# dcaustin33/intro_to_gaussian_splatting

Measured on AMD Instinct MI355X. Metric: Mpixels/sec forward raster (1M Gaussians, 1080p) + max |dpixel| vs CPU ref, higher is better.
Workload: dtype f32; 1 GPU; C3: synthetic 1M Gaussians, 1920x1080 (metric config); n_gaussians=1000000, width=1920, height=1080, tile=16, semantics=ref_cpu, layout=wh3, frames_in_flight=1, launch=one hipGraph replay per frame, frame_sync=speculative (GSX_FLAG_NO_SYNC), counts confirmed after the timed region, parallelism=1 GPU

## Files before the change

### intro_to_gaussian_splatting_amd/csrc/gsx_api.hip

```cpp
#include <float.h>
#include <math.h>
#include <stdarg.h>
#include <stdio.h>
#include <string.h>

#include "gsx_internal.h"
#ifdef GSX_TEST_HOOKS
#include "gsx_debug.h"
#endif

namespace {

thread_local char g_error[512] = "";

int fail(int code, const char *fmt, ...) {
    va_list ap;
    va_start(ap, fmt);
    vsnprintf(g_error, sizeof g_error, fmt, ap);
    va_end(ap);
    return code;
}

#define GSX_HIP(expr)                                                                               \
    do {                                                                                            \
// ... 85 lines not shown
                     bool &sampled) {
    uint32_t *k0 = (uint32_t *)(ws + c.keys0), *k1 = (uint32_t *)(ws + c.keys1);
    uint32_t *v0 = (uint32_t *)(ws + c.vals0), *v1 = (uint32_t *)(ws + c.vals1);
    uint32_t *counters = (uint32_t *)(ws + c.counters);
    const uint32_t *row_of = p.original_index ? (const uint32_t *)p.row_of_index : nullptr;
    const gsx::DepthRoute route = gsx::depth_sort_route(n, p.kept_hint);
    sampled = route != gsx::kDepthLsd;
    gsx::SortHints sh{nullptr, nullptr, nullptr, false};
    gsx::ScheduleHint sched_hint{nullptr, nullptr, nullptr, 0u};
    if (fh && p.hints && (route == gsx::kDepth256 || route == gsx::kDepthLsd) && n >= gsx::kSortSamples && p.grid.count() > 0 &&
        gsx::blend_splits_long_tiles(p.grid, p.semantics, p.generic)) {
        const gsx::HintsLayout hl = gsx::hints_layout(max_tiles_of(p.grid.width, p.grid.height, p.grid.tile),
                                                      max_axis_tiles_of(p.grid.width, p.grid.height, p.grid.tile));
        uint32_t *hdr = (uint32_t *)p.hints;
        sh = gsx::SortHints{hdr, (const uint32_t *)(p.hints + hl.splitters), (uint32_t *)(p.hints + hl.samples),
                            p.hints_valid && route == gsx::kDepth256};
        const bool exact = route == gsx::kDepth256 && gsx::knob("GSX_EXACT_SPLITTERS", 1) != 0;
        if (exact) sh.next_splitters = (uint32_t *)(p.hints + hl.splitters);
        fh->blend = gsx::BlendHints{hdr, exact ? nullptr : sh.samples, (uint32_t *)(p.hints + hl.splitters), (uint32_t *)(p.hints + hl.lens), 0u};
        fh->sched_region = (uint32_t *)(p.hints + hl.sched);
        if (p.hints_valid && p.schedule != 0 && p.grid.count() > 2048) {
            sched_hint = gsx::ScheduleHint{(const uint32_t *)(p.hints + hl.lens), (uint32_t *)(p.hints + hl.sched), hdr,
                                           (uint32_t)p.grid.count(), (uint32_t)p.grid.nwy()};
            fh->sched = sched_hint.sched;
        }
    }
    gsx::SampleHint presample;
    if (sampled && !sh.use && gsx::knob("GSX_PRESAMPLE", 1) != 0)
        presample = gsx::depth_presample(route, ws + c.temp, n, gsx::emit_chunk_sums(ws + c.temp, n, cap), row_of);
    GSX_HIP(gsx::launch_project_pack(camera, p.camera_device, in, n, p.grid, p.semantics, p.tight, p.small_batch, p.sh_degree, k0, (gsx::Record *)(ws + c.rec),
                                     (gsx::TileRect *)(ws + c.rect), counters,
                                     p.semantics != GSX_SEM_STD_3DGS ? (float4 *)(ws + c.bbox) : nullptr, sched_hint,
                                     c.temp_bytes >= (size_t)(n / GSX_BOUNDS_ROWS + 1) ? (uint8_t *)(ws + c.temp) : nullptr, s, presample));
    if (tm) tm->mark();
    if (sampled)
        GSX_HIP(gsx::sort_depth_sampled(route, ws + c.temp, k0, k1, v0, v1, n, p.kept_hint, counters + kCtrKept,
                                        counters + kCtrCulled, (const gsx::TileRect *)(ws + c.rect),
                                        (gsx::TileRect *)(ws + c.rrect), 0, gsx::emit_chunk_sums(ws + c.temp, n, cap), sh, s, row_of,
                                        presample.splitters != nullptr));
    else {
        const bool carry = p.grid.ntx <= 256 && p.grid.nty <= 256 && cap >= n && gsx::knob("GSX_LSD_CARRY", 1) != 0;
        GSX_HIP(gsx::sort_depth_compact(ws + c.temp, k0, k1, v0, v1, n, counters + kCtrKept, counters + kCtrCulled,
                                        (const gsx::TileRect *)(ws + c.rect), (gsx::TileRect *)(ws + c.rrect), s, sh.samples,
                                        carry ? (uint32_t *)(ws + c.tvals0) : nullptr,
                                        carry ? (uint32_t *)(ws + c.tvals1) : nullptr, row_of));
    }
    if (tm) tm->mark();
    order = v0;
    return GSX_OK;
}

int bin_pairs(const Plan &p, const Carve &c, char *ws, int64_t n, int64_t cap, const gsx::TileRect *rrect,
              const uint32_t *order, const uint32_t *m_dev, bool sums_ready, const gsx::BinCounts &bc,
              const gsx::LongTiles &lt, StageTimer *tm, hipStream_t s, const uint32_t *&sorted_vals) {
    uint2 *ranges = (uint2 *)(ws + c.ranges);
    GSX_HIP(gsx::emit_instances(ws + c.temp, rrect, order, m_dev, n, cap, p.grid, ws + c.tkeys0, (uint32_t *)(ws + c.tvals0),
                                ranges, bc, sums_ready, p.kept_hint, s));
    if (tm) tm->mark();
    if (p.grid.count() > 0)
        GSX_HIP(gsx::sort_instances(ws + c.temp, cap, p.grid, ws + c.tkeys0, ws + c.tkeys1, (uint32_t *)(ws + c.tvals0),
                                    (uint32_t *)(ws + c.tvals1), ranges, bc.d32, lt, &sorted_vals, s));
    return GSX_OK;
}

int read_counts(const Carve &c, char *ws, int64_t cap, bool on_device, uint32_t *redo, int64_t (&counts)[3], hipStream_t s) {
    counts[0] = counts[1] = counts[2] = 0;
    if (on_device) GSX_HIP(hipMemcpyAsync(counts, ws + c.counters + 16, 24, hipMemcpyDeviceToHost, s));
    if (redo) GSX_HIP(hipMemcpyAsync(redo, ws + c.redo, 4, hipMemcpyDeviceToHost, s));
    GSX_HIP(hipStreamSynchronize(s));
    if (counts[1] > cap)
        return fail(GSX_ERR_WORKSPACE_TOO_SMALL, "frame needs %lld tile instances, workspace holds %lld",
                    (long long)counts[1], (long long)cap);
    return GSX_OK;
}

int bin_and_blend(const Plan &p, const Carve &c, char *ws, int64_t n, int64_t cap, const gsx::TileRect *rrect,
                  const uint32_t *order, const uint32_t *m_dev, const uint32_t *culled_dev, bool sums_ready,
                  GsxFrameStats *stats, StageTimer &tm, hipStream_t s, const FrameHints &fh = FrameHints()) {
    uint32_t *counters = (uint32_t *)(ws + c.counters);
    int64_t *dev2 = (int64_t *)(counters + 4);
    uint2 *ranges = (uint2 *)(ws + c.ranges);
    bool counts_on_device = false, counts_in_host = false;
    bool redo_counted = false;
    const bool has_redo = p.stats_bytes >= offsetof(GsxFrameStats, n_redo) + sizeof(int64_t);
    if (p.plain && !stats) return fail(GSX_ERR_INVALID_ARGUMENT, "GSX_FLAG_PLAIN_FOOTPRINTS needs stats_host: n_redo must reach the caller");
    bool parts_marked = false;
    if (n == 0 && p.tile_counts && p.grid.count() > 0)
        GSX_HIP(gsx::launch_zero_words(p.tile_counts, (size_t)p.grid.count(), s));
    if (p.grid.count() > 0 && n == 0 && p.semantics == GSX_SEM_STD_3DGS) {
        tm.mark();
        GSX_HIP(gsx::launch_zero_words((uint32_t *)ranges, (size_t)p.grid.count() * 2, s));
        GSX_HIP(gsx::launch_blend((const gsx::Record *)(ws + c.rec), nullptr, (const uint32_t *)(ws + c.tvals0), ranges,
                                  p.grid, p.out, p.semantics, p.background, p.generic, make_clear_plan(p, false),
                                  gsx::LongTiles{nullptr, nullptr, 0u}, nullptr, gsx::BlendHints{nullptr, nullptr, nullptr, nullptr, 0u}, s));
    } else if (n == 0) {
        tm.mark();
        GSX_HIP(gsx::launch_clear(make_clear_plan(p, true), p.out.ptr, s));
    } else {
        gsx::BinCounts bc{dev2, nullptr, counters + kCtrPairs, counters + kCtrLong, (uint32_t *)(ws + c.redo), culled_dev, n};
        if (p.no_sync && stats) {
            void *alias = nullptr;
            if (hipHostGetDevicePointer(&alias, stats, 0) == hipSuccess && alias) {
                bc.stats2_host = (int64_t *)alias;
                counts_in_host = true;
            } else {
                (void)hipGetLastError();
            }
        }
        const bool split = p.split && cap > 0 && gsx::blend_splits_long_tiles(p.grid, p.semantics, p.generic);
        gsx::LongTiles lt{counters + kCtrLong, (uint32_t *)(ws + c.longs), split ? gsx::kMaxLongTiles : 0u};
        lt.redo = (uint32_t *)(ws + c.redo);
        if (fh.blend.lens) {
            lt.cost = fh.blend.lens;
            lt.header = fh.blend.header;
            lt.cost_pct = (uint32_t)gsx::knob("GSX_LONG_COST_PCT", 30);
            lt.stay_pct = (uint32_t)gsx::knob("GSX_LONG_STAY_PCT", 75);
            if (!fh.sched || lt.cost_pct == 0) lt.header = nullptr;
        }
        const uint32_t *sorted_vals = nullptr;
        const int rc = bin_pairs(p, c, ws, n, cap, rrect, order, m_dev, sums_ready, bc, lt, &tm, s, sorted_vals);
        if (rc != GSX_OK) return rc;
        counts_on_device = true;
        if (p.grid.count() == 0) {
            GSX_HIP(gsx::launch_clear(make_clear_plan(p, true), p.out.ptr, s));
        } else {
            if (p.tile_counts) GSX_HIP(gsx::launch_tile_counts(ranges, p.grid.count(), p.tile_counts, s));
            const uint32_t *sched = fh.sched;
            gsx::BlendHints bh = fh.blend;
            bh.xcd_sched = fh.sched ? 1u : 0u;
            if (!sched && cap > 0 && gsx::blend_uses_schedule(p.grid, p.semantics, p.generic, n, p.schedule)) {
                if (p.semantics == GSX_SEM_REF_CPU && gsx::knob("GSX_COLD_XCD_SCHED", 1) != 0) {
                    uint32_t *hdr = bh.header ? bh.header : (uint32_t *)(ws + c.sched_header);
                    uint32_t *region = (bh.header && fh.sched_region) ? fh.sched_region : (uint32_t *)(ws + c.sched);
                    if (!(bh.header && !fh.sched_region)) {
                        GSX_HIP(gsx::launch_tile_schedule_xcd(ranges, p.grid.count(), p.grid.nwy(), region, hdr, s));
                        sched = region;
                        bh.header = hdr;
                        bh.xcd_sched = 1u;
                    }
                }
                if (!sched) {
                    sched = (uint32_t *)(ws + c.sched);
                    GSX_HIP(gsx::launch_tile_schedule(ranges, p.grid.count(), (uint32_t *)(ws + c.sched), s));
                }
            }
            tm.mark();
            bh.plain = p.plain ? 1u : 0u;
            redo_counted = p.semantics == GSX_SEM_REF_CPU && p.grid.tile == 16 && !p.generic;
            const int64_t ntl = p.grid.count();
            bh.rank_last = (fh.sched && ntl > 7400 && ntl <= 8192 && (int64_t)cap >= 128 * ntl) ? 1u : 0u;
            if (gsx::knob("GSX_RANK_LAST", -1) >= 0) bh.rank_last = (uint32_t)gsx::knob("GSX_RANK_LAST", -1);
            if (p.n_parts > 1 && gsx::blend_in_parts(p.grid, p.semantics, p.generic)) {
                bool first = true;
                for (int k = 0; k < p.n_parts; ++k) {
                    const gsx::TileSpan span{p.part_axis, p.part_bounds[k], p.part_bounds[k + 1], first ? 1u : 0u, (uint32_t)k};
                    if (span.hi > span.lo || (first && k == p.n_parts - 1)) {
                        GSX_HIP(gsx::launch_blend((const gsx::Record *)(ws + c.rec), (const float4 *)(ws + c.bbox), sorted_vals,
                                                  ranges, p.grid, p.out, p.semantics, p.background, p.generic,
                                                  make_clear_plan(p, false), lt, sched, bh, s, &span));
                        first = false;
                    }
                    GSX_HIP(hipEventRecord((hipEvent_t)p.part_events[k], s));
                }
                parts_marked = true;
            } else {
                GSX_HIP(gsx::launch_blend((const gsx::Record *)(ws + c.rec), (const float4 *)(ws + c.bbox), sorted_vals,
                                          ranges, p.grid, p.out, p.semantics, p.background, p.generic,
                                          make_clear_plan(p, false), lt, sched, bh, s));
            }
            tm.mark();
        }
    }
    if (!parts_marked)
        for (int k = 0; k < p.n_parts; ++k) GSX_HIP(hipEventRecord((hipEvent_t)p.part_events[k], s));
    if (p.no_sync) {
        if (stats) {
            if (!counts_on_device) {
                stats->n_visible = 0;
                stats->n_instances = 0;
                stats->n_kept = 0;
            } else if (!counts_in_host) {
                GSX_HIP(hipMemcpyAsync(stats, dev2, 16, hipMemcpyDeviceToHost, s));
                GSX_HIP(hipMemcpyAsync(&stats->n_kept, dev2 + 2, 8, hipMemcpyDeviceToHost, s));
            }
            if (has_redo) {
                stats->n_redo = 0;
                if (redo_counted) GSX_HIP(hipMemcpyAsync(&stats->n_redo, ws + c.redo, 4, hipMemcpyDeviceToHost, s));
            }
            stats->n_tiles = p.grid.count();
            stats->reserved = cap;
        }
        return GSX_OK;
    }
    int64_t host2[3];
    uint32_t redo_host = 0;
    const int rc = read_counts(c, ws, cap, counts_on_device, redo_counted ? &redo_host : nullptr, host2, s);
    if (rc != GSX_OK && rc != GSX_ERR_WORKSPACE_TOO_SMALL) return rc;
    if (stats) {
        stats->n_visible = host2[0];
        stats->n_instances = host2[1];
        stats->n_kept = host2[2];
        if (has_redo) stats->n_redo = redo_host;
        stats->n_tiles = p.grid.count();
        stats->reserved = 0;
    }
    tm.finish(stats);
    return rc;
}

#ifdef GSX_TEST_HOOKS
thread_local float g_backward_ms[3] = {0.0f, 0.0f, 0.0f};
#endif

struct GeometryGrads {
    float *means3d, *scales, *quats;
};

int render_backward(const GsxCamera *camera, const float *means3d, const float *scales, const float *quats,
                    const float *opacity_logit, const float *colors, int64_t n, int32_t tile_size, const float *image,
                    const float *grad_image, float *grad_colors, float *grad_opacity_logit, const GeometryGrads *geo,
                    const GsxParams *params, void *workspace, size_t workspace_bytes, void *stream) {
    hipStream_t s = (hipStream_t)stream;
    if (!camera) return fail(GSX_ERR_INVALID_ARGUMENT, "camera is NULL");
    Plan p;
    int rc = make_plan_or_fail(camera->width, camera->height, tile_size, const_cast<float *>(image), params, p);
    if (rc != GSX_OK) return rc;
    if (p.semantics != GSX_SEM_REF_CPU) return fail(GSX_ERR_INVALID_ARGUMENT, "gsx_render_backward supports GSX_SEM_REF_CPU only");
    if (p.sh) return fail(GSX_ERR_INVALID_ARGUMENT, "gsx_render_backward takes RGB colours, not GsxParams.sh");
    if (p.grid.wx0 != 0 || p.grid.wy0 != 0 || p.grid.wx1 != p.grid.ntx || p.grid.wy1 != p.grid.nty)
        return fail(GSX_ERR_INVALID_ARGUMENT, "gsx_render_backward renders the whole frame: no tile window");
    if (p.out.x0 != 0 || p.out.y0 != 0 || p.out.w != camera->width || p.out.h != camera->height)
        return fail(GSX_ERR_INVALID_ARGUMENT, "gsx_render_backward takes the whole frame: no output window");
    if (p.n_parts > 0) return fail(GSX_ERR_INVALID_ARGUMENT, "gsx_render_backward does not take substrips");
    if (params && (params->flags & GSX_FLAG_NO_SYNC)) return fail(GSX_ERR_INVALID_ARGUMENT, "gsx_render_backward synchronises: no GSX_FLAG_NO_SYNC");
    if (p.camera_device) return fail(GSX_ERR_INVALID_ARGUMENT, "gsx_render_backward reads the camera argument: no camera_device");
    rc = check_inputs(p, n, means3d, scales, quats, opacity_logit, colors);
    if (rc != GSX_OK) return rc;
    if (!grad_image || !grad_colors || !grad_opacity_logit) return fail(GSX_ERR_INVALID_ARGUMENT, "grad_image / grad_colors / grad_opacity_logit is NULL");
    Carve c;
    int64_t cap;
    rc = check_workspace(workspace, workspace_bytes, n, max_tiles_of(camera->width, camera->height, tile_size), c, cap,
                         geo ? kCarveGeometry : kCarveBackward);
    if (rc != GSX_OK) return rc;
    char *ws = (char *)workspace;
    StageTimer tm;
    tm.begin(p.timing, s);
    GSX_HIP(gsx::launch_zero_words((uint32_t *)grad_colors, (size_t)n * 3, s));
    GSX_HIP(gsx::launch_zero_words((uint32_t *)grad_opacity_logit, (size_t)n, s));
    if (geo) {
        GSX_HIP(gsx::launch_zero_words((uint32_t *)geo->means3d, (size_t)n * 3, s));
        GSX_HIP(gsx::launch_zero_words((uint32_t *)geo->scales, (size_t)n * 3, s));
        GSX_HIP(gsx::launch_zero_words((uint32_t *)geo->quats, (size_t)n * 4, s));
    }
    if (n == 0 || p.grid.count() == 0) {
        GSX_HIP(hipStreamSynchronize(s));
        return GSX_OK;
    }
    const gsx::GaussiansIn in{means3d, scales, quats, opacity_logit, colors, p.original_index, nullptr};
    const uint32_t *order;
    bool sampled;
    rc = project_and_sort(p, c, ws, *camera, in, n, cap, nullptr, nullptr, s, order, sampled);
    if (rc != GSX_OK) return rc;
    uint32_t *counters = (uint32_t *)(ws + c.counters);
    const gsx::TileRect *rrect = (const gsx::TileRect *)(ws + c.rrect);
    const gsx::BinCounts bcnt{(int64_t *)(counters + 4), nullptr, counters + kCtrPairs, counters + kCtrLong,
                              (uint32_t *)(ws + c.redo), counters + kCtrCulled, n};
    const gsx::LongTiles lt{counters + kCtrLong, (uint32_t *)(ws + c.longs), 0u};
    const uint32_t *sorted_vals = nullptr;
    rc = bin_pairs(p, c, ws, n, cap, rrect, order, counters + kCtrKept, sampled, bcnt, lt, nullptr, s, sorted_vals);
    if (rc != GSX_OK) return rc;
// ... 447 lines not shown
```

### intro_to_gaussian_splatting_amd/csrc/gsx_binning.hip

```cpp

#include "gsx_internal.h"
#include "gsx_schedule_device.h"

namespace gsx {
namespace {

constexpr int kBlock = 256;
constexpr int kPerThread = 4;
constexpr int kChunk = kBlock * kPerThread;
static_assert(kChunk == kEmitChunk, "gsx_plan.h sizes the chunk sums with this");
constexpr int kSelfScanChunks = 2048;

__device__ __forceinline__ void load_rects(const TileRect *__restrict__ rrect, uint32_t first, uint32_t m,
                                           TileRect (&r)[kPerThread]) {
    if (first + kPerThread <= m) {
        const uint4 *src = reinterpret_cast<const uint4 *>(rrect + first);
        const uint4 a = src[0], b = src[1];
        const uint32_t w[8] = {a.x, a.y, a.z, a.w, b.x, b.y, b.z, b.w};
#pragma unroll
        for (int k = 0; k < kPerThread; ++k) {
            r[k].x0 = (uint16_t)(w[2 * k] & 0xFFFFu);
            r[k].x1 = (uint16_t)(w[2 * k] >> 16);
            r[k].y0 = (uint16_t)(w[2 * k + 1] & 0xFFFFu);
            r[k].y1 = (uint16_t)(w[2 * k + 1] >> 16);
// ... 92 lines not shown
    uint32_t end;
};

template <typename Key, bool PREFIXED>
__global__ void __launch_bounds__(kBlock)
    emit_kernel(const TileRect *__restrict__ rrect, const uint32_t *__restrict__ order,
                const uint32_t *__restrict__ m_dev, uint32_t bound, const uint64_t *__restrict__ sums, int nchunks,
                TileGrid g, uint32_t limit, Key *__restrict__ keys, uint32_t *__restrict__ vals,
                uint2 *__restrict__ ranges, EmitCounts ec, uint32_t eager) {
    __shared__ uint64_t wsum[4];
    __shared__ uint32_t offs[kChunk + 1];
    __shared__ __attribute__((aligned(16))) EmitSlot slot[kChunk + 2];
    {
        const int64_t t = (int64_t)blockIdx.x * kBlock + threadIdx.x;
        if (t < g.count()) ranges[t] = make_uint2(0u, 0u);
    }
    if ((int)blockIdx.x >= nchunks) return;
    const int lane = threadIdx.x & 63, w = threadIdx.x >> 6;
    const uint32_t first = blockIdx.x * (uint32_t)kChunk + threadIdx.x * (uint32_t)kPerThread;

    TileRect r[kPerThread];
    uint32_t gidx[kPerThread];
    const bool early = blockIdx.x * (uint32_t)kChunk < eager;
    uint32_t m = 0;
    if (!early) m = load_count(m_dev, bound);
    const uint32_t fetch_bound = early ? bound : m;
    load_rects(rrect, first, fetch_bound, r);
#pragma unroll
    for (int k = 0; k < kPerThread; ++k) gidx[k] = first + k < fetch_bound ? (order ? order[first + k] : first + k) : 0u;
    if (early) m = load_count(m_dev, bound);
    uint64_t base;
    const bool last = (int)blockIdx.x == nchunks - 1;
    if (PREFIXED) {
        base = sums[blockIdx.x];
    } else {
        uint64_t before = 0;
        for (int k = threadIdx.x; k < (int)blockIdx.x; k += kBlock) before += sums[k];
        base = block_sum64(before, wsum);
    }

    uint32_t c[kPerThread];
    uint64_t mine = 0;
#pragma unroll
    for (int k = 0; k < kPerThread; ++k) {
        c[k] = first + k < m ? tiles_of(r[k]) : 0u;
        mine += c[k];
    }
    uint64_t x = mine;
#pragma unroll
    for (int o = 1; o < 64; o <<= 1) {
        const uint64_t y = (uint64_t)__shfl_up((long long)x, o);
        if (lane >= o) x += y;
    }
    if (lane == 63) wsum[w] = x;
    __syncthreads();
    uint64_t run = x - mine;
    for (int k = 0; k < w; ++k) run += wsum[k];
    const uint64_t chunk_total = wsum[0] + wsum[1] + wsum[2] + wsum[3];
    auto sat = [](uint64_t v) -> uint32_t { return v > 0xFFFFFFFFull ? 0xFFFFFFFFu : (uint32_t)v; };
#pragma unroll
    for (int k = 0; k < kPerThread; ++k) {
        offs[threadIdx.x * kPerThread + k] = sat(run);
        run += c[k];
        slot[threadIdx.x * kPerThread + k] = EmitSlot{(uint32_t)r[k].x0 | ((uint32_t)r[k].x1 << 16),
                                                      (uint32_t)r[k].y0 | ((uint32_t)r[k].y1 << 16), gidx[k], sat(run)};
    }
    if (threadIdx.x == kBlock - 1) offs[kChunk] = sat(run);
    if (threadIdx.x < 2) slot[kChunk + threadIdx.x] = EmitSlot{0u, 0u, 0u, 0xFFFFFFFFu};
    __syncthreads();

    if (last && threadIdx.x == 0) {
        const uint64_t d = PREFIXED ? sums[nchunks] : base + chunk_total;
        const int64_t nvis = ec.n_total - (ec.culled_dev ? (int64_t)*ec.culled_dev : 0);
        ec.stats2[0] = nvis;
        ec.stats2[1] = (int64_t)d;
        ec.stats2[2] = (int64_t)m;
        if (ec.stats2_host) {
            ec.stats2_host[0] = nvis;
            ec.stats2_host[1] = (int64_t)d;
            ec.stats2_host[7] = (int64_t)m;
        }
        *ec.d32 = d > 0xFFFFFFFFull ? 0xFFFFFFFFu : (uint32_t)d;
        *ec.long_count = 0u;
        *ec.redo_count = 0u;
    }

    if (base >= (uint64_t)limit) return;
    const uint64_t room = (uint64_t)limit - base;
    const uint32_t npairs = (uint32_t)(chunk_total < room ? chunk_total : room);
    if (npairs == 0) return;
    const uint32_t out0 = (uint32_t)base, out1 = out0 + npairs;
    const uint32_t nwy = (uint32_t)g.nwy();
    const uint32_t q_first = out0 & ~7u;
    const uint32_t groups = (out1 - q_first + 7u) >> 3;
    const uint4 *slots = reinterpret_cast<const uint4 *>(slot);
    for (uint32_t gi = threadIdx.x; gi < groups; gi += (uint32_t)kBlock) {
        const uint32_t qb = q_first + gi * 8u;
        const uint32_t qa = max(qb, out0), qe = min(qb + 8u, out1);
        uint32_t p = qa - out0;
        uint32_t lo = 0, hi = kChunk;
#pragma unroll
        for (int s_ = 0; s_ < 10; ++s_) {
            const uint32_t mid = (lo + hi) >> 1;
            const bool right = offs[mid] <= p;
            lo = right ? mid : lo;
            hi = right ? hi : mid;
        }
        uint4 cur = slots[lo], ahead = slots[lo + 1];
        uint32_t x0 = cur.x & 0xFFFFu, y0 = cur.y & 0xFFFFu, y1 = cur.y >> 16;
        uint32_t tx, ty;
        {
            const uint32_t k = p - offs[lo], h = y1 - y0 + 1u;
            tx = x0 + k / h;
            ty = y0 + k % h;
        }
        uint32_t key = (tx - (uint32_t)g.wx0) * nwy + (ty - (uint32_t)g.wy0);
        for (uint32_t q8 = qb; q8 < qe; q8 += 8u) {
            uint32_t kk[8], vv[8];
#pragma unroll
            for (uint32_t i = 0; i < 8u; ++i) {
                const uint32_t q = q8 + i;
                kk[i] = key;
                vv[i] = cur.z;
                if (q >= qa && q + 1u < qe) {
                    ++p;
                    if (p >= cur.w) {
                        do {
                            cur = ahead;
                            ++lo;
                            ahead = slots[lo + 1];
                        } while (p >= cur.w);
                        x0 = cur.x & 0xFFFFu;
                        y0 = cur.y & 0xFFFFu;
                        y1 = cur.y >> 16;
                        tx = x0;
                        ty = y0;
                        key = (tx - (uint32_t)g.wx0) * nwy + (ty - (uint32_t)g.wy0);
                    } else if (ty == y1) {
                        ty = y0;
                        ++tx;
                        key += nwy - (y1 - y0);
                    } else {
                        ++ty;
                        ++key;
                    }
                }
            }
            if (q8 >= qa && q8 + 8u <= qe) {
                if (sizeof(Key) == 2) {
                    *reinterpret_cast<uint4 *>(keys + q8) =
                        make_uint4(kk[0] | (kk[1] << 16), kk[2] | (kk[3] << 16), kk[4] | (kk[5] << 16), kk[6] | (kk[7] << 16));
                } else {
                    uint4 *dk = reinterpret_cast<uint4 *>(keys + q8);
                    dk[0] = make_uint4(kk[0], kk[1], kk[2], kk[3]);
                    dk[1] = make_uint4(kk[4], kk[5], kk[6], kk[7]);
                }
                uint4 *dv = reinterpret_cast<uint4 *>(vals + q8);
                dv[0] = make_uint4(vv[0], vv[1], vv[2], vv[3]);
                dv[1] = make_uint4(vv[4], vv[5], vv[6], vv[7]);
            } else {
#pragma unroll
                for (uint32_t i = 0; i < 8u; ++i) {
                    const uint32_t q = q8 + i;
                    if (q >= qa && q < qe) {
                        keys[q] = (Key)kk[i];
                        vals[q] = vv[i];
                    }
                }
// ... 257 lines not shown
```

### intro_to_gaussian_splatting_amd/csrc/gsx_blend.hip

```cpp
#include <type_traits>

#include "gsx_internal.h"
#include "gsx_schedule_device.h"

namespace gsx {
namespace {

constexpr uint32_t kBatchCost = 5;
constexpr int kPad = 8;
constexpr int kBlocks = 4;
template <int BATCH>
struct __attribute__((aligned(16))) StagedT {
    static constexpr int kBatch = BATCH, kSlots = BATCH + kPad, kNull = BATCH;
    static constexpr bool kWide = BATCH > 64;
    float4 rec[3][kSlots];
    uint16_t list[kBlocks][kSlots];
};
using Staged = StagedT<64>;
using StagedWide = StagedT<128>;
static_assert(sizeof(StagedWide) >= sizeof(Staged) && alignof(StagedWide) == alignof(Staged), "the REF kernel's helpers stage 64 records in the same LDS");
static_assert((StagedWide::kSlots - 1) * 16 <= 0xFFFF, "list entries are 16-bit byte offsets");

__device__ __forceinline__ uint32_t xcd_remap(uint32_t b, uint32_t n) {
    uint32_t xcd = b & 7u, i = b >> 3, q = n >> 3, r = n & 7u;
// ... 711 lines not shown
                    }
                    const uint32_t s0_ = my_list[k], s1_ = my_list[k + 1];
                    const bool r0 = is_ref(s0_), r1 = is_ref(s1_);
                    if (!__any(r0 | r1)) {
                        exact_pair();
                        continue;
                    }
                    const float4 A0 = *reinterpret_cast<const float4 *>(rec_a + s0_), B0 = *reinterpret_cast<const float4 *>(rec_b + s0_);
                    const float2 C0 = *reinterpret_cast<const float2 *>(rec_c + s0_);
                    v2f aa, ab, ta_a, ta_b;
                    if (r0)
                        alphas_ref(A0, B0.x, C0.y, B0.y, fx_, fya, fyb, aa, ab);
                    else
                        alphas(A0, B0.x, B0.y, cx, cya, cyb, aa, ab);
                    checked_pair(aa, Ta, ta_a);
                    checked_pair(ab, Tb, ta_b);
                    GSX_ACCUMULATE(ta_a, ta_b, B0.z, B0.w, C0.x);
                    k += 1;
                }
            }
        }
        tile_sync<REF>();
        const unsigned long long alive = __ballot((Ta.x > 0.0f) | (Ta.y > 0.0f) | (Tb.x > 0.0f) | (Tb.y > 0.0f));
        if (alive == 0ull) break;
        if (checked) {
#pragma unroll
            for (int gb = 0; gb < kBlocks; ++gb) dead |= (alive & lanes_of[gb]) == 0ull ? (1u << gb) : 0u;
        }
    }
    if (restart_scalar) {
        tile_sync<REF>();
        Staged &sh64 = reinterpret_cast<Staged &>(sh);
#pragma unroll
        for (int j = 0; j < 4; ++j) {
            T[j] = 1.0f;
            c0[j] = c1[j] = c2[j] = 0.0f;
        }
#pragma unroll
        for (int gb = 0; gb < kBlocks; ++gb) skipped[gb] = 0u;
        for (uint32_t base = rg.x; base < rg.y; base += 64) {
            uint32_t nb = (uint32_t)__builtin_amdgcn_readfirstlane((int)min(64u, rg.y - base));
            uint32_t count[kBlocks];
            const int later = stage_batch<kStageBlocks, REF>(rec, qraw, vals, base, nb, sh64, lane, (float)(tx * 16), (float)(ty * 16),
                                                             16.0f, skipped, count, budget);
            if (REF && (later & kBatchHasRef)) saw_ref = true;
            if (!REF && (later & kBatchKindMask) >= kBatchRefOrder) {
                if (lane == 0) atomicAdd(lt.redo, 1u);
                return;
            }
            cost += 4u * nb;
            tile_sync<REF>();
            for (uint32_t k = 0; k < nb; ++k) {
                const Splat s = read_splat(sh64, k);
                composite<4, REF>(cx, cy, s, T, c0, c1, c2, blk, (float)(tx * 16), (float)(ty * 16));
            }
            tile_sync<REF>();
            if (__ballot((T[0] > 0.0f) | (T[1] > 0.0f) | (T[2] > 0.0f) | (T[3] > 0.0f)) == 0ull) break;
        }
    } else {
        c0[0] = c0a.x; c0[1] = c0a.y; c0[2] = c0b.x; c0[3] = c0b.y;
        c1[0] = c1a.x; c1[1] = c1a.y; c1[2] = c1b.x; c1[3] = c1b.y;
        c2[0] = c2a.x; c2[1] = c2a.y; c2[2] = c2b.x; c2[3] = c2b.y;
    }

    if (hints.lens && lane == 0) hints.lens[t] = cost;
    if (REF && saw_ref && lane == 0 && lt.redo) atomicAdd(lt.redo, 1u);
    float *o = out.ptr + (int64_t)(px - out.x0) * out.stride_x + (int64_t)(py0 - out.y0) * out.stride_y;
    if (y_contig && (reinterpret_cast<uintptr_t>(o) & 15u) == 0) {
        float4 *o4 = reinterpret_cast<float4 *>(o);
        o4[0] = make_float4(c0[0], c1[0], c2[0], c0[1]);
        o4[1] = make_float4(c1[1], c2[1], c0[2], c1[2]);
        o4[2] = make_float4(c2[2], c0[3], c1[3], c2[3]);
    } else {
#pragma unroll
        for (int j = 0; j < 4; ++j) {
            float *oj = o + (int64_t)j * out.stride_y;
            oj[0] = c0[j];
            oj[1] = c1[j];
            oj[2] = c2[j];
        }
    }
}

template <bool REF, class SH>
__device__ __forceinline__ void blend_tile16_grid(const Record *__restrict__ rec, const float4 *__restrict__ qraw,
                                                  const uint32_t *__restrict__ vals, const uint2 *__restrict__ ranges,
                                                  const TileGrid &g, const OutDesc &out, const ClearPlan &cp, const LongTiles &lt,
                                                  uint32_t nhelpers, const uint32_t *__restrict__ sched, uint32_t budget,
                                                  const BlendHints &hints, uint32_t tile_blocks, uint32_t sched_cap_,
                                                  const TileSpan &span, SH &sh) {
    const uint32_t nrank = hints.samples ? kRankGroups : 0u;
    const uint32_t rank0 = hints.rank_last ? gridDim.x - nrank : 0u;
    if (blockIdx.x - rank0 < nrank) {
        if (span.first) rank_samples(blockIdx.x - rank0, (int)threadIdx.x, hints);
        return;
    }
    const uint32_t block = hints.rank_last ? blockIdx.x : blockIdx.x - nrank;
    if (block < nhelpers) {
        const uint32_t b = block, slot = (b >> 5) * 8u + (b & 7u);
        const int quarter = (int)((b >> 3) & 3u);
        if (slot >= min(*lt.count, lt.max)) return;
        const uint32_t lt_tile = lt.list[slot];
        {
            const int lead = span.axis ? g.wy0 + (int)(lt_tile % (uint32_t)g.nwy()) : g.wx0 + (int)(lt_tile / (uint32_t)g.nwy());
            if (lead < span.lo || lead >= span.hi) return;
        }
        blend_long_tile_quarter<REF>(rec, qraw, vals, ranges, g, out, lt_tile, quarter, reinterpret_cast<Staged &>(sh), budget,
                                     hints.lens ? hints.lens + lt_tile : nullptr, lt.redo);
        return;
    }
    const uint32_t bid = block - nhelpers;
    if (bid >= tile_blocks) {
        if (span.first) clear_block(bid - tile_blocks, cp, out.ptr);
        return;
    }
    const uint32_t t = hints.xcd_sched ? xcd_scheduled_tile(bid, (uint32_t)g.count(), sched_cap_, sched, hints.header)
                                       : scheduled_tile(bid, (uint32_t)g.count(), sched);
    if (t >= (uint32_t)g.count()) return;
    blend_tile16<REF, SH>(rec, qraw, vals, ranges, g, out, lt, budget, hints, span, t, sh);
}

#ifndef GSX_PLAIN_WAVES
#define GSX_PLAIN_WAVES 8
#endif
__global__ void __launch_bounds__(64) __attribute__((amdgpu_waves_per_eu(GSX_PLAIN_WAVES, 8)))
    blend_tile16_kernel(const Record *__restrict__ rec, const float4 *__restrict__ qraw, const uint32_t *__restrict__ vals,
                        const uint2 *__restrict__ ranges, TileGrid g, OutDesc out, ClearPlan cp, LongTiles lt,
                        uint32_t nhelpers, const uint32_t *__restrict__ sched, uint32_t budget, BlendHints hints,
                        uint32_t tile_blocks, uint32_t sched_cap_, TileSpan span) {
    __shared__ Staged sh;
    blend_tile16_grid<false, Staged>(rec, qraw, vals, ranges, g, out, cp, lt, nhelpers, sched, budget, hints, tile_blocks, sched_cap_, span, sh);
}

#ifndef GSX_REF_WAVES
#define GSX_REF_WAVES 4
#endif
__global__ void __launch_bounds__(64) __attribute__((amdgpu_waves_per_eu(GSX_REF_WAVES, 8)))
    blend_tile16_ref_kernel(const Record *__restrict__ rec, const float4 *__restrict__ qraw, const uint32_t *__restrict__ vals,
                            const uint2 *__restrict__ ranges, TileGrid g, OutDesc out, ClearPlan cp, LongTiles lt,
                            uint32_t nhelpers, const uint32_t *__restrict__ sched, uint32_t budget, BlendHints hints,
                            uint32_t tile_blocks, uint32_t sched_cap_, TileSpan span) {
    __shared__ StagedWide sh;
    blend_tile16_grid<true, StagedWide>(rec, qraw, vals, ranges, g, out, cp, lt, nhelpers, sched, budget, hints, tile_blocks, sched_cap_, span, sh);
}

__global__ void __launch_bounds__(64)
    blend_generic_kernel(const Record *__restrict__ rec, const float4 *__restrict__ qraw, const uint32_t *__restrict__ vals,
                         const uint2 *__restrict__ ranges, TileGrid g, OutDesc out, ClearPlan cp) {
    __shared__ Staged sh;
    if (blockIdx.x >= (uint32_t)g.count()) {
        clear_block(blockIdx.x - (uint32_t)g.count(), cp, out.ptr);
        return;
    }
    const int lane = threadIdx.x;
    const uint32_t t = xcd_remap(blockIdx.x, (uint32_t)g.count());
    const int tx = g.wx0 + (int)(t / (uint32_t)g.nwy()), ty = g.wy0 + (int)(t % (uint32_t)g.nwy());
    const int Ts = g.tile, npx = Ts * Ts;
    const uint2 rg = ranges[t];
    const bool fast_y = out.stride_y < out.stride_x;
    const bool blocks = Ts == 16;
    for (int chunk = 0; chunk < npx; chunk += 64) {
        uint32_t skipped[kBlocks] = {0u, 0u, 0u, 0u}, count[kBlocks];
        const int p = chunk + lane;
        const bool valid = p < npx;
        const int pf = p % Ts, ps = p / Ts;
        const int lx = fast_y ? ps : pf, ly = fast_y ? pf : ps;
        const int px = tx * Ts + lx, py = ty * Ts + ly;
        const float fx = (float)lx, fy = (float)ly;
        const int blk = blocks ? ((lx >> 3) | ((ly >> 3) << 1)) & 3 : 0;
        float T[1] = {1.0f}, c0[1] = {0.0f}, c1[1] = {0.0f}, c2[1] = {0.0f};
        for (uint32_t base = rg.x; base < rg.y; base += 64) {
            uint32_t nb = min(64u, rg.y - base);
            if (blocks)
                (void)stage_batch<kStageBlocks>(rec, qraw, vals, base, nb, sh, lane, (float)(tx * Ts), (float)(ty * Ts), (float)Ts, skipped, count);
            else
                (void)stage_batch<kStageWhole>(rec, qraw, vals, base, nb, sh, lane, (float)(tx * Ts), (float)(ty * Ts), (float)Ts, skipped, count);
            __syncthreads();
            for (uint32_t k = 0; k < nb; ++k) {
                const Splat s = read_splat(sh, k);
                const float e_p[1] = {fy};
                composite<1>(fx, e_p, s, T, c0, c1, c2, blk, (float)(tx * Ts), (float)(ty * Ts));
            }
            __syncthreads();
            if (__ballot(valid && T[0] > 0.0f) == 0ull) break;
        }
        if (valid) {
            float *o = out.ptr + (int64_t)(px - out.x0) * out.stride_x + (int64_t)(py - out.y0) * out.stride_y;
            o[0] = c0[0];
            o[1] = c1[0];
            o[2] = c2[0];
        }
    }
}

constexpr float kStdAlphaMin = 1.0f / 255.0f, kStdStop = 0.0001f;

__device__ __forceinline__ void std_composite(float pw, float alpha, float cr, float cg, float cb, float &thr, float &T,
                                              float &c0, float &c1, float &c2) {
    const bool use = !(pw > 0.0f) && !(alpha < thr);
    const float ta = T * alpha;
    const bool stop = use && (T - ta < kStdStop);
    const float w = (use && !stop) ? ta : 0.0f;
    thr = stop ? __builtin_inff() : thr;
    c0 = __builtin_fmaf(w, cr, c0);
    c1 = __builtin_fmaf(w, cg, c1);
    c2 = __builtin_fmaf(w, cb, c2);
    T = T - w;
}

template <int SEM>
__global__ void __launch_bounds__(64)
    blend_rules_kernel(const Record *__restrict__ rec, const float4 *__restrict__ bbox,
                       const uint32_t *__restrict__ vals, const uint2 *__restrict__ ranges, TileGrid g,
                       OutDesc out, float bg0, float bg1, float bg2, ClearPlan cp) {
    __shared__ float4 sh[4][64];
    if (blockIdx.x >= (uint32_t)g.count()) {
        clear_block(blockIdx.x - (uint32_t)g.count(), cp, out.ptr);
        return;
    }
    const int lane = threadIdx.x;
    const uint32_t t = xcd_remap(blockIdx.x, (uint32_t)g.count());
    const int tx = g.wx0 + (int)(t / (uint32_t)g.nwy()), ty = g.wy0 + (int)(t % (uint32_t)g.nwy());
    const int Ts = g.tile, npx = Ts * Ts;
    const uint2 rg = ranges[t];
    const bool fast_y = out.stride_y < out.stride_x;
    for (int chunk = 0; chunk < npx; chunk += 64) {
// ... 283 lines not shown
```

### intro_to_gaussian_splatting_amd/csrc/gsx_internal.h

```cpp
#pragma once

#include <hip/hip_runtime.h>
#include <stdint.h>
#include <stdlib.h>

#include "gsx.h"
#include "gsx_plan.h"

namespace gsx {

inline int knob(const char *name, int dflt) {
#ifdef GSX_TEST_HOOKS
    const char *e = getenv(name);
    return e && *e ? atoi(e) : dflt;
#else
    (void)name;
    return dflt;
#endif
}

constexpr uint32_t kCulledKey = 0xFFFFFFFFu;
constexpr uint32_t kEmptyKey = 0xFFFFFFFEu;

struct __attribute__((aligned(16))) Record {
    float4 a, b, c;
};
static_assert(sizeof(Record) == kRecordBytes, "gsx_plan.h sizes the workspace with this");

struct TileRect {
    uint16_t x0, x1, y0, y1;
};
static_assert(sizeof(TileRect) == kTileRectBytes && sizeof(float4) == kBboxBytes && sizeof(uint2) == kRangeBytes,
              "gsx_plan.h sizes the workspace with these");

__device__ __forceinline__ uint32_t tiles_of(const TileRect &r) {
    return r.x0 > r.x1 ? 0u : (uint32_t)(r.x1 - r.x0 + 1) * (uint32_t)(r.y1 - r.y0 + 1);
}

__device__ __forceinline__ uint32_t load_count(const uint32_t *n_dev, uint32_t bound) {
    if (!n_dev) return bound;
    const uint32_t n = *n_dev;
    return n < bound ? n : bound;
}

constexpr float kStopRefCpu = 0.000001f;

__device__ __forceinline__ float alpha_ref(float x, float y, float q00, float q01, float q10, float q11, float op,
                                           float px, float py) {
    const float e0 = x - px, e1 = y - py;
    const float d0 = -0.5f * e0, d1 = -0.5f * e1;
    const float t0 = __builtin_fmaf(d1, q10, d0 * q00);
    const float t1 = __builtin_fmaf(d1, q11, d0 * q01);
    const float power = t0 * e0 + t1 * e1;
    return __builtin_amdgcn_exp2f(power * 1.44269504088896340736f) * op;
}

__device__ __forceinline__ float alpha_ref_tail(float x, float y, float q00, float q01, float q10, float q11, float op,
                                                float px, float py, float alpha) {
    const float e0 = x - px, e1 = y - py;
    const float d0 = -0.5f * e0, d1 = -0.5f * e1;
    const float t0 = __builtin_fmaf(d1, q10, d0 * q00);
    const float t1 = __builtin_fmaf(d1, q11, d0 * q01);
    const float p2 = (t0 * e0 + t1 * e1) * 1.44269504088896340736f;
    return p2 < -100.0f ? (__builtin_amdgcn_exp2f(p2 + 64.0f) * op) * 0x1p-64f : alpha;
}

constexpr uint32_t kLongFlag = 0x80000000u;
struct LongTiles {
    uint32_t *count;
    uint32_t *list;
    uint32_t max;
    uint32_t *cost = nullptr;
    const uint32_t *header = nullptr;
    uint32_t cost_pct = 30;
    uint32_t stay_pct = 75;
    uint32_t *redo = nullptr;
};
__host__ __device__ inline uint32_t long_tile_threshold(uint32_t pairs, uint32_t tiles) {
    const uint32_t mean = tiles ? pairs / tiles : 0u;
    const uint32_t four = mean > 0x3FFFFFFFu ? 0xFFFFFFFFu : 4u * mean;
    return four > 1024u ? four : 1024u;
}

struct StageOneOut {
    float *points_xy, *colors, *cov2d, *depths, *inv_cov, *radius, *min_x, *max_x, *min_y, *max_y, *sig_op;
    int32_t *order;
};

struct GaussiansIn {
    const float *means3d, *scales, *quats, *opacity_logit, *colors;
    const int32_t *original_index = nullptr;
    const float4 *block_bounds = nullptr;
};

struct PreprocessedIn {
    const float *means, *colors, *inv_cov, *min_x, *max_x, *min_y, *max_y, *opacity;
};

struct ScheduleHint {
    const uint32_t *lens;
    uint32_t *sched, *header;
    uint32_t ntiles, nwy;
};

hipError_t launch_project_stage(const GsxCamera &cam, const GaussiansIn &in, int64_t n, uint32_t *keys, Record *stage,
                                uint32_t *counters, int visible_rows, hipStream_t s);
struct SampleHint {
    uint32_t *splitters = nullptr;
    unsigned long long *chunk_sums = nullptr;
    uint32_t nsums = 0, ns = 0;
    const uint32_t *row_of = nullptr;
};
hipError_t launch_project_pack(const GsxCamera &cam, const GsxCamera *cam_device, const GaussiansIn &in, int64_t n,
                               const TileGrid &grid, int semantics, bool tight_rects, int visible_rows, int sh_degree,
                               uint32_t *keys, Record *rec, TileRect *rect, uint32_t *counters, float4 *bbox,
                               const ScheduleHint &sched, uint8_t *block_scratch, hipStream_t s,
                               const SampleHint &sample = SampleHint());
hipError_t launch_project_full(const Record *stage, const uint32_t *order, const uint32_t *m_dev, int64_t n,
                               const StageOneOut &out, hipStream_t s);
hipError_t launch_pack_preprocessed(const PreprocessedIn &in, int64_t n, const TileGrid &grid, int semantics,
                                    Record *rec, TileRect *rect, float4 *bbox, hipStream_t s);
hipError_t launch_project_raw(const GsxCamera &cam, const GaussiansIn &in, int64_t n, int visible_rows, Record *raw, hipStream_t s);
hipError_t launch_covariance3d(const float *scales, const float *quats, int64_t n, float *out, hipStream_t s);
hipError_t launch_covariance2d(const GsxCamera &cam, const float *points, const float *cov3d, int64_t n, float *out,
                               hipStream_t s);
hipError_t launch_project_points(const GsxCamera &cam, const float *means3d, int64_t n, float *points_out,
                                 uint8_t *in_view, hipStream_t s);

struct BinCounts {
    int64_t *stats2;
    int64_t *stats2_host;
    uint32_t *d32;
    uint32_t *long_count;
    uint32_t *redo_count;
    const uint32_t *culled_dev;
    int64_t n_total;
};
hipError_t emit_instances(void *temp, const TileRect *rrect, const uint32_t *order, const uint32_t *m_dev, int64_t n,
                          int64_t cap, const TileGrid &grid, void *keys0, uint32_t *vals0, uint2 *ranges,
                          const BinCounts &bc, bool sums_ready, int64_t kept_hint, hipStream_t s);
hipError_t sort_instances(void *temp, int64_t cap, const TileGrid &grid, void *keys0, void *keys1, uint32_t *vals0,
                          uint32_t *vals1, uint2 *ranges, const uint32_t *d32, const LongTiles &lt,
                          const uint32_t **sorted_vals, hipStream_t s);
hipError_t launch_tile_counts(const uint2 *ranges, int64_t nt, uint32_t *counts, hipStream_t s);
hipError_t launch_tile_schedule(const uint2 *ranges, int64_t nt, uint32_t *sched, hipStream_t s);
hipError_t launch_tile_schedule_xcd(const uint2 *ranges, int64_t nt, int64_t nwy, uint32_t *sched, uint32_t *header, hipStream_t s);
hipError_t radix_sort_pairs_u32(void *temp, uint32_t *&keys_cur, uint32_t *&keys_alt, uint32_t *&vals_cur,
                                uint32_t *&vals_alt, const uint32_t *n_dev, int64_t bound, int key_bits,
                                hipStream_t s);
hipError_t radix_sort_pairs_u16(void *temp, uint16_t *&keys_cur, uint16_t *&keys_alt, uint32_t *&vals_cur,
                                uint32_t *&vals_alt, const uint32_t *n_dev, int64_t bound, int key_bits,
                                hipStream_t s);
hipError_t sort_depth_compact(void *temp, uint32_t *keys0, uint32_t *keys1, uint32_t *&vals_cur, uint32_t *&vals_alt,
                              int64_t n, uint32_t *m_dev, uint32_t *culled_dev, const TileRect *rect, TileRect *rrect,
                              hipStream_t s, uint32_t *samples_out = nullptr, uint32_t *carry0 = nullptr,
                              uint32_t *carry1 = nullptr, const uint32_t *row_of = nullptr);

enum DepthRoute { kDepthLsd = 0, kDepth256 = 1, kDepth1024 = 2, kDepthOneWorkgroup = 3 };
DepthRoute depth_sort_route(int64_t n, int64_t kept_hint);
// ... 136 lines not shown
```

### intro_to_gaussian_splatting_amd/csrc/gsx_plan.h

```cpp
#pragma once

#include <stdarg.h>
#include <stddef.h>
#include <stdint.h>
#include <stdio.h>
#include <string.h>

#include "gsx.h"

#if defined(__HIPCC__)
#define GSX_HD __host__ __device__
#else
#define GSX_HD
#endif

namespace gsx {

constexpr int kSortItems = 2048;
constexpr int kSortQuad = 4;
constexpr int kSortBins = 256;
constexpr int kEmitChunk = 1024;
constexpr uint32_t kMaxLongTiles = 512;
constexpr int kMaxSubstrips = 16;
constexpr size_t kParamsBytesAbi300 = 104;
constexpr int kClearFloats = 6144;
constexpr size_t kRecordBytes = 48, kTileRectBytes = 8, kBboxBytes = 16, kRangeBytes = 8;

struct TileGrid {
    int32_t tile, ntx, nty;
    int32_t wx0, wx1, wy0, wy1;
    int32_t width, height;
    GSX_HD int32_t nwx() const { return wx1 - wx0; }
    GSX_HD int32_t nwy() const { return wy1 - wy0; }
    GSX_HD int64_t count() const { return (int64_t)nwx() * nwy(); }
};

struct OutDesc {
    float *ptr;
    int64_t stride_x, stride_y;
    int32_t x0, y0, w, h;
};

struct ClearPlan {
    int32_t n;
    int32_t first[5];
    int32_t s0[4], f0[4], rows[4], fw[4];
    int64_t pitch;
};


constexpr int kSortBinsMax = 1024;
constexpr int kSortSamples = 2048, kSortSamplesMax = 8192, kSortQuadTotals = 64;
inline size_t radix_temp_bytes(int64_t max_items, int bins = kSortBins) {
    const size_t nblocks = (size_t)((max_items + kSortItems - 1) / kSortItems) + 9 * kSortQuad;
    return ((size_t)bins * (nblocks + kSortQuad) + 2 * (size_t)bins + (size_t)kSortQuadTotals * kSortBins) * sizeof(uint32_t);
}
inline size_t binning_sums_offset(int64_t n, int64_t cap) {
    const int64_t items = n > cap ? n : cap;
    const size_t a = radix_temp_bytes(items > 1 ? items : 1);
    const size_t b = radix_temp_bytes(n > 1 ? n : 1, kSortBinsMax);
    return ((a > b ? a : b) + 255) & ~(size_t)255;
}
inline size_t binning_temp_bytes(int64_t n, int64_t cap) {
    const size_t nchunks = (size_t)((n + kEmitChunk - 1) / kEmitChunk) + 2;
    return binning_sums_offset(n, cap) + ((nchunks * sizeof(uint64_t) + 255) & ~(size_t)255);
}
inline int clear_blocks_for(int64_t rows, int64_t fw) {
    const int64_t floats = rows * fw * 3;
    return (int)((floats + kClearFloats - 1) / kClearFloats);
}

enum { kHintSplitters = 0, kHintSamples = 1, kHintLens = 2, kHintSched = 3, kHintLongPct = 4, kHintXcdTiles = 8 ,
       kHintXcdCost = 16 , kHintHeaderWords = 64 };
constexpr uint32_t kSchedXcds = 8;
struct SchedCut {
    uint32_t k, s, rem;
};
GSX_HD inline SchedCut sched_cut(uint32_t nt) {
    SchedCut c;
    c.k = nt / (kSchedXcds * 32u) ? nt / (kSchedXcds * 32u) : 1u;
    c.s = nt / (kSchedXcds * c.k);
    c.rem = nt - c.s * kSchedXcds * c.k;
    return c;
}
GSX_HD inline uint32_t sched_cap(uint32_t nt, uint32_t ) {
    const SchedCut c = sched_cut(nt);
    return (c.s + 1u) * c.k;
}
struct HintsLayout {
    size_t splitters, samples, lens, sched, total;
};
inline size_t hints_sched_entries(int64_t max_tiles) {
    const size_t t = (size_t)(max_tiles > 0 ? max_tiles : 1);
    return t + t / 32 + 64;
}
inline HintsLayout hints_layout(int64_t max_tiles, int64_t ) {
    HintsLayout h;
    const size_t t = (size_t)(max_tiles > 0 ? max_tiles : 1);
    h.splitters = kHintHeaderWords * 4;
    h.samples = h.splitters + (size_t)kSortBins * 4;
    h.lens = h.samples + (size_t)kSortSamples * 4;
    h.sched = h.lens + ((t * 4 + 255) & ~(size_t)255);
    h.total = h.sched + ((hints_sched_entries(max_tiles) * 4 + 255) & ~(size_t)255);
    return h;
}

namespace plan {

constexpr size_t kAlign = 256;
constexpr int64_t kMaxPairs = ((int64_t)1 << 31) - 1;
inline size_t align_up(size_t v) { return (v + kAlign - 1) & ~(kAlign - 1); }

inline void default_params(GsxParams *params, size_t bytes = sizeof(GsxParams)) {
    if (bytes > sizeof(GsxParams)) bytes = sizeof(GsxParams);
    if (bytes < kParamsBytesAbi300) bytes = kParamsBytesAbi300;
    GsxParams d;
    memset(&d, 0, sizeof d);
    d.struct_size = (int32_t)bytes;
    d.semantics = GSX_SEM_REF_CPU;
    d.layout = GSX_LAYOUT_WH3;
    d.tile_x1 = -1;
    d.tile_y1 = -1;
    d.stats_size = (int32_t)sizeof(GsxFrameStats);
    memcpy(params, &d, bytes);
}

inline const int32_t *original_index_of(const GsxParams *params) {
    if (!params) return nullptr;
    const size_t have = params->struct_size ? (size_t)params->struct_size : kParamsBytesAbi300;
    return have >= offsetof(GsxParams, original_index) + sizeof(const int32_t *) ? params->original_index : nullptr;
}

inline int32_t tiles_along(int32_t extent, int32_t tile, int semantics) {
    if (semantics == GSX_SEM_REF_CPU) return extent > tile ? (extent - tile + tile - 1) / tile : 0;
    return (extent + tile - 1) / tile;
}

struct Carve {
    size_t keys0, keys1, vals0, vals1;
    size_t rec, rect, rrect, bbox;
    size_t tkeys0, tkeys1, tvals0, tvals1;
    size_t ranges, longs, redo, sched_header, sched, counters, temp, temp_bytes, total;
    size_t raw, rank_of, prefix, bsum, slots;
    size_t geo_slots;
};

enum { kCarveForward = 0, kCarveBackward = 1, kCarveGeometry = 2 };
constexpr size_t kGeoSlotBytes = 32;

enum { kCtrCulled = 0, kCtrKept = 1, kCtrPairs = 2, kCtrLong = 3 };

inline Carve carve(int64_t n, int64_t cap, int64_t max_tiles, size_t temp_bytes, int backward = kCarveForward) {
    Carve c = {};
    size_t off = 0;
    auto take = [&](size_t bytes) {
        size_t at = off;
        off = align_up(off + bytes);
        return at;
    };
    size_t nn = (size_t)(n > 0 ? n : 1), cc = (size_t)(cap > 0 ? cap : 1);
    c.keys0 = take(nn * 4); c.keys1 = take(nn * 4); c.vals0 = take(nn * 4); c.vals1 = take(nn * 4);
    c.rec = take(nn * kRecordBytes);
    c.rect = take(nn * kTileRectBytes);
    c.rrect = take(nn * kTileRectBytes);
    c.bbox = take(nn * kBboxBytes);
    c.tkeys0 = take(cc * 4); c.tkeys1 = take(cc * 4); c.tvals0 = take(cc * 4); c.tvals1 = take(cc * 4);
    c.ranges = take((size_t)(max_tiles > 0 ? max_tiles : 1) * kRangeBytes);
    c.longs = take(kMaxLongTiles * sizeof(uint32_t));
    c.redo = take(256);
    c.sched_header = take(kHintHeaderWords * sizeof(uint32_t));
    c.sched = take(hints_sched_entries(max_tiles) * sizeof(uint32_t));
    c.counters = take(64);
    c.temp = take(temp_bytes);
    c.temp_bytes = temp_bytes;
    if (backward) {
        c.raw = take(nn * kRecordBytes);
        c.rank_of = take(nn * 4);
        c.prefix = take((nn + 1) * 4);
        c.bsum = take((nn / 1024 + 2) * 4);
        c.slots = take(cc * 16);
    }
    if (backward == kCarveGeometry) c.geo_slots = take(cc * kGeoSlotBytes);
    c.total = off;
    return c;
}

constexpr int kLossTile = 32;
constexpr int kLossHalo = 5;
struct LossCarve {
    int64_t tiles_r, tiles_c, tiles, map_stride;
    size_t partials, maps[3], total;
};
inline bool loss_carve(int32_t rows, int32_t cols, bool with_grad, LossCarve &c) {
    c = LossCarve{};
    if (rows <= 0 || cols <= 0) return false;
    c.tiles_r = ((int64_t)rows + kLossTile - 1) / kLossTile;
    c.tiles_c = ((int64_t)cols + kLossTile - 1) / kLossTile;
    c.tiles = c.tiles_r * c.tiles_c;
    if (c.tiles > kMaxPairs) return false;
    c.map_stride = ((int64_t)cols * 3 + 3) & ~(int64_t)3;
    size_t off = 0;
    auto take = [&](size_t bytes) {
        size_t at = off;
        off = align_up(off + bytes);
        return at;
    };
    c.partials = take((size_t)c.tiles * 2 * sizeof(float));
    if (with_grad)
        for (int k = 0; k < 3; ++k) c.maps[k] = take((size_t)rows * (size_t)c.map_stride * sizeof(float));
    c.total = off;
    return true;
}

inline int64_t max_tiles_of(int32_t width, int32_t height, int32_t tile) {
    return (int64_t)((width + tile - 1) / tile) * ((height + tile - 1) / tile);
}
inline int64_t max_axis_tiles_of(int32_t width, int32_t height, int32_t tile) {
    const int64_t a = (width + tile - 1) / tile, b = (height + tile - 1) / tile;
    return a > b ? a : b;
}

inline int64_t capacity_for(size_t bytes, int64_t n, int64_t max_tiles, int backward = kCarveForward) {
    auto fits = [&](int64_t cap) { return carve(n, cap, max_tiles, binning_temp_bytes(n, cap), backward).total <= bytes; };
    if (!fits(1)) return -1;
    int64_t lo = 1, hi = kMaxPairs;
    if (fits(hi)) return hi;
    while (hi - lo > 1) {
        const int64_t mid = lo + (hi - lo) / 2;
        if (fits(mid))
            lo = mid;
        else
            hi = mid;
    }
    return lo;
}

struct Plan {
    TileGrid grid;
    OutDesc out;
    int semantics;
    bool timing;
    bool no_sync;
    bool generic;
    bool tight;
    bool split;
    bool plain;
    size_t stats_bytes;
    int small_batch;
    int schedule;
    const GsxCamera *camera_device;
    uint32_t *tile_counts;
    const float *sh;
// ... 168 lines not shown
```

Before: 6213 Mpixels/s.

## Publish redo count to mapped host memory from last finishing blend block

Result: no change. 6222 Mpixels/s (median of 4 runs) (+0.1%).

```diff
diff --git a/intro_to_gaussian_splatting_amd/csrc/gsx_api.hip b/intro_to_gaussian_splatting_amd/csrc/gsx_api.hip
--- a/intro_to_gaussian_splatting_amd/csrc/gsx_api.hip
+++ b/intro_to_gaussian_splatting_amd/csrc/gsx_api.hip
@@ -191,6 +191,8 @@
     uint2 *ranges = (uint2 *)(ws + c.ranges);
     bool counts_on_device = false, counts_in_host = false;
     bool redo_counted = false;
+    bool redo_in_host = false;
+    int64_t *redo_alias = nullptr;
     const bool has_redo = p.stats_bytes >= offsetof(GsxFrameStats, n_redo) + sizeof(int64_t);
     if (p.plain && !stats) return fail(GSX_ERR_INVALID_ARGUMENT, "GSX_FLAG_PLAIN_FOOTPRINTS needs stats_host: n_redo must reach the caller");
     bool parts_marked = false;
@@ -212,6 +214,7 @@
             if (hipHostGetDevicePointer(&alias, stats, 0) == hipSuccess && alias) {
                 bc.stats2_host = (int64_t *)alias;
                 counts_in_host = true;
+                if (has_redo) redo_alias = (int64_t *)((char *)alias + offsetof(GsxFrameStats, n_redo));
             } else {
                 (void)hipGetLastError();
             }
@@ -273,6 +276,10 @@
                 }
                 parts_marked = true;
             } else {
+                if (redo_counted && redo_alias) {
+                    lt.redo_host = redo_alias;
+                    redo_in_host = true;
+                }
                 GSX_HIP(gsx::launch_blend((const gsx::Record *)(ws + c.rec), (const float4 *)(ws + c.bbox), sorted_vals,
                                           ranges, p.grid, p.out, p.semantics, p.background, p.generic,
                                           make_clear_plan(p, false), lt, sched, bh, s));
@@ -294,7 +301,7 @@
             }
             if (has_redo) {
                 stats->n_redo = 0;
-                if (redo_counted) GSX_HIP(hipMemcpyAsync(&stats->n_redo, ws + c.redo, 4, hipMemcpyDeviceToHost, s));
+                if (redo_counted && !redo_in_host) GSX_HIP(hipMemcpyAsync(&stats->n_redo, ws + c.redo, 4, hipMemcpyDeviceToHost, s));
             }
             stats->n_tiles = p.grid.count();
             stats->reserved = cap;
diff --git a/intro_to_gaussian_splatting_amd/csrc/gsx_binning.hip b/intro_to_gaussian_splatting_amd/csrc/gsx_binning.hip
--- a/intro_to_gaussian_splatting_amd/csrc/gsx_binning.hip
+++ b/intro_to_gaussian_splatting_amd/csrc/gsx_binning.hip
@@ -198,8 +198,8 @@
         }
         *ec.d32 = d > 0xFFFFFFFFull ? 0xFFFFFFFFu : (uint32_t)d;
         *ec.long_count = 0u;
-        *ec.redo_count = 0u;
-    }
+    }
+    if (last && threadIdx.x <= kRedoWords) reinterpret_cast<uint64_t *>(ec.redo_count)[threadIdx.x] = 0ull;
 
     if (base >= (uint64_t)limit) return;
     const uint64_t room = (uint64_t)limit - base;
diff --git a/intro_to_gaussian_splatting_amd/csrc/gsx_blend.hip b/intro_to_gaussian_splatting_amd/csrc/gsx_blend.hip
--- a/intro_to_gaussian_splatting_amd/csrc/gsx_blend.hip
+++ b/intro_to_gaussian_splatting_amd/csrc/gsx_blend.hip
@@ -817,42 +817,63 @@
     }
 }
 
+constexpr uint32_t kNoFinish = 0xFFFFFFFFu;
+__device__ __forceinline__ uint32_t *redo_word(const LongTiles &lt, uint32_t f) {
+    return lt.redo_host ? lt.redo + 2u * (1u + (f & (kRedoWords - 1u))) : lt.redo;
+}
+__device__ __forceinline__ void redo_finish(const LongTiles &lt, uint32_t f, uint32_t nhelpers, uint32_t tile_blocks) {
+    if (!lt.redo_host || f == kNoFinish || threadIdx.x != 0) return;
+    unsigned long long *root = reinterpret_cast<unsigned long long *>(lt.redo);
+    const uint32_t nlong = nhelpers ? min(*lt.count, lt.max) : 0u;
+    const uint32_t w = f & (kRedoWords - 1u);
+    const uint32_t mine = (tile_blocks + kRedoWords - 1u - w) / kRedoWords + 4u * ((nlong + kRedoWords - 1u - w) / kRedoWords);
+    const unsigned long long a = atomicAdd(root + 1 + w, 1ull << 32);
+    if ((uint32_t)(a >> 32) + 1u != mine) return;
+    const uint32_t words = min(max(tile_blocks, nlong), kRedoWords);
+    const unsigned long long b = atomicAdd(root, (1ull << 32) | (a & 0xFFFFFFFFull));
+    if ((uint32_t)(b >> 32) + 1u != words) return;
+    *lt.redo_host = (int64_t)((uint32_t)b + (uint32_t)a);
+}
+
 template <bool REF, class SH>
-__device__ __forceinline__ void blend_tile16_grid(const Record *__restrict__ rec, const float4 *__restrict__ qraw,
-                                                  const uint32_t *__restrict__ vals, const uint2 *__restrict__ ranges,
-                                                  const TileGrid &g, const OutDesc &out, const ClearPlan &cp, const LongTiles &lt,
-                                                  uint32_t nhelpers, const uint32_t *__restrict__ sched, uint32_t budget,
-                                                  const BlendHints &hints, uint32_t tile_blocks, uint32_t sched_cap_,
-                                                  const TileSpan &span, SH &sh) {
+__device__ __forceinline__ uint32_t blend_tile16_grid(const Record *__restrict__ rec, const float4 *__restrict__ qraw,
+                                                      const uint32_t *__restrict__ vals, const uint2 *__restrict__ ranges,
+                                                      const TileGrid &g, const OutDesc &out, const ClearPlan &cp, const LongTiles &lt,
+                                                      uint32_t nhelpers, const uint32_t *__restrict__ sched, uint32_t budget,
+                                                      const BlendHints &hints, uint32_t tile_blocks, uint32_t sched_cap_,
+                                                      const TileSpan &span, SH &sh) {
     const uint32_t nrank = hints.samples ? kRankGroups : 0u;
     const uint32_t rank0 = hints.rank_last ? gridDim.x - nrank : 0u;
     if (blockIdx.x - rank0 < nrank) {
         if (span.first) rank_samples(blockIdx.x - rank0, (int)threadIdx.x, hints);
-        return;
+        return kNoFinish;
     }
     const uint32_t block = hints.rank_last ? blockIdx.x : blockIdx.x - nrank;
     if (block < nhelpers) {
         const uint32_t b = block, slot = (b >> 5) * 8u + (b & 7u);
         const int quarter = (int)((b >> 3) & 3u);
-        if (slot >= min(*lt.count, lt.max)) return;
+        if (slot >= min(*lt.count, lt.max)) return kNoFinish;
         const uint32_t lt_tile = lt.list[slot];
         {
             const int lead = span.axis ? g.wy0 + (int)(lt_tile % (uint32_t)g.nwy()) : g.wx0 + (int)(lt_tile / (uint32_t)g.nwy());
-            if (lead < span.lo || lead >= span.hi) return;
+            if (lead < span.lo || lead >= span.hi) return slot;
         }
         blend_long_tile_quarter<REF>(rec, qraw, vals, ranges, g, out, lt_tile, quarter, reinterpret_cast<Staged &>(sh), budget,
-                                     hints.lens ? hints.lens + lt_tile : nullptr, lt.redo);
-        return;
+                                     hints.lens ? hints.lens + lt_tile : nullptr, redo_word(lt, slot));
+        return slot;
     }
     const uint32_t bid = block - nhelpers;
     if (bid >= tile_blocks) {
         if (span.first) clear_block(bid - tile_blocks, cp, out.ptr);
-        return;
+        return kNoFinish;
     }
     const uint32_t t = hints.xcd_sched ? xcd_scheduled_tile(bid, (uint32_t)g.count(), sched_cap_, sched, hints.header)
                                        : scheduled_tile(bid, (uint32_t)g.count(), sched);
-    if (t >= (uint32_t)g.count()) return;
-    blend_tile16<REF, SH>(rec, qraw, vals, ranges, g, out, lt, budget, hints, span, t, sh);
+    if (t >= (uint32_t)g.count()) return bid;
+    LongTiles l = lt;
+    l.redo = redo_word(lt, bid);
+    blend_tile16<REF, SH>(rec, qraw, vals, ranges, g, out, l, budget, hints, span, t, sh);
+    return bid;
 }
 
 #ifndef GSX_PLAIN_WAVES
@@ -864,7 +885,8 @@
                         uint32_t nhelpers, const uint32_t *__restrict__ sched, uint32_t budget, BlendHints hints,
                         uint32_t tile_blocks, uint32_t sched_cap_, TileSpan span) {
     __shared__ Staged sh;
-    blend_tile16_grid<false, Staged>(rec, qraw, vals, ranges, g, out, cp, lt, nhelpers, sched, budget, hints, tile_blocks, sched_cap_, span, sh);
+    const uint32_t f = blend_tile16_grid<false, Staged>(rec, qraw, vals, ranges, g, out, cp, lt, nhelpers, sched, budget, hints, tile_blocks, sched_cap_, span, sh);
+    redo_finish(lt, f, nhelpers, tile_blocks);
 }
 
 #ifndef GSX_REF_WAVES
@@ -876,7 +898,8 @@
                             uint32_t nhelpers, const uint32_t *__restrict__ sched, uint32_t budget, BlendHints hints,
                             uint32_t tile_blocks, uint32_t sched_cap_, TileSpan span) {
     __shared__ StagedWide sh;
-    blend_tile16_grid<true, StagedWide>(rec, qraw, vals, ranges, g, out, cp, lt, nhelpers, sched, budget, hints, tile_blocks, sched_cap_, span, sh);
+    const uint32_t f = blend_tile16_grid<true, StagedWide>(rec, qraw, vals, ranges, g, out, cp, lt, nhelpers, sched, budget, hints, tile_blocks, sched_cap_, span, sh);
+    redo_finish(lt, f, nhelpers, tile_blocks);
 }
 
 __global__ void __launch_bounds__(64)
diff --git a/intro_to_gaussian_splatting_amd/csrc/gsx_internal.h b/intro_to_gaussian_splatting_amd/csrc/gsx_internal.h
--- a/intro_to_gaussian_splatting_amd/csrc/gsx_internal.h
+++ b/intro_to_gaussian_splatting_amd/csrc/gsx_internal.h
@@ -75,6 +75,7 @@
     uint32_t cost_pct = 30;
     uint32_t stay_pct = 75;
     uint32_t *redo = nullptr;
+    int64_t *redo_host = nullptr;
 };
 __host__ __device__ inline uint32_t long_tile_threshold(uint32_t pairs, uint32_t tiles) {
     const uint32_t mean = tiles ? pairs / tiles : 0u;
diff --git a/intro_to_gaussian_splatting_amd/csrc/gsx_plan.h b/intro_to_gaussian_splatting_amd/csrc/gsx_plan.h
--- a/intro_to_gaussian_splatting_amd/csrc/gsx_plan.h
+++ b/intro_to_gaussian_splatting_amd/csrc/gsx_plan.h
@@ -21,6 +21,7 @@
 constexpr int kSortBins = 256;
 constexpr int kEmitChunk = 1024;
 constexpr uint32_t kMaxLongTiles = 512;
+constexpr uint32_t kRedoWords = 64;
 constexpr int kMaxSubstrips = 16;
 constexpr size_t kParamsBytesAbi300 = 104;
 constexpr int kClearFloats = 6144;
@@ -167,7 +168,7 @@
     c.tkeys0 = take(cc * 4); c.tkeys1 = take(cc * 4); c.tvals0 = take(cc * 4); c.tvals1 = take(cc * 4);
     c.ranges = take((size_t)(max_tiles > 0 ? max_tiles : 1) * kRangeBytes);
     c.longs = take(kMaxLongTiles * sizeof(uint32_t));
-    c.redo = take(256);
+    c.redo = take((kRedoWords + 1) * sizeof(uint64_t));
     c.sched_header = take(kHintHeaderWords * sizeof(uint32_t));
     c.sched = take(hints_sched_entries(max_tiles) * sizeof(uint32_t));
     c.counters = take(64);
```
